# manonkok/Rao-Blackwellized-SLAM-smoothing

Measured on AMD Instinct MI355X. Metric: particle-steps/s (filter) + smoother wall-clock, N=65k T=3k, higher is better.
Workload: dtype f64

## Files before the change

include/rbpf.h:

```cpp
#ifndef RBPF_H_
#define RBPF_H_

#include <stddef.h>
#include <stdint.h>

#ifdef __cplusplus
extern "C" {
#endif

#define RBPF_ABI_VERSION 9

typedef enum {
  RBPF_OK = 0,
  RBPF_ERR_INVALID_ARG = 1,
  RBPF_ERR_UNSUPPORTED = 2,
  RBPF_ERR_HIP = 3,
  RBPF_ERR_NO_DEVICE = 4,
  RBPF_ERR_OUT_OF_MEMORY = 5,
  RBPF_ERR_CHOL_FAILED = 6,
  RBPF_ERR_STATE = 7,
  RBPF_ERR_CALLBACK = 8
} rbpf_status;

typedef enum {
// ... 213 lines not shown
                   int32_t n_p, const double* xn, const double* odo, double dt, const double* Q,
                   const double* z, double* xn_next);
int rbpf_dyn_res_norm(const rbpf_model* model, int32_t n_nonlin, int32_t n_w, int32_t n_odo,
                      int32_t n_p, const double* xnk_t, const double* xn, const double* odo,
                      double dt, const double* Q, double* e_dyn);
int rbpf_sample(int32_t N, const double* w, int32_t n_draws, const double* u, int32_t* ind);
int rbpf_jacobian_phi3d(const rbpf_model* model, int32_t n_p, const double* x,
                        const double* lower, const double* upper, double* J);
int rbpf_chol_weights(int32_t M, int32_t batch, const double* S, const double* e, double jitter,
                      int32_t variant, int32_t reps, double* logw, int32_t* status, double* ms);
int32_t rbpf_chol_refresh_resolve(int32_t model_kind, int32_t n_lin, int32_t n_y, int32_t requested);
int rbpf_chol_sweep_probe(int32_t n, int32_t d, int32_t batch, const double* L, const double* U, const double* V,
                          const double* eta, int32_t reps, double* L_out, double* logw, int32_t* status, double* ms);
int rbpf_quat_helpers(int32_t op, int32_t n, const double* in, double* out);
int rbpf_probe_wave_reduce(const double* in, double* out);

typedef struct {
  int32_t struct_size;
  int32_t m_basis;
  const int32_t* NN;
  double L[3];
  const double* mean;
  const double* V;
  double sigma2;
  const double* var_table;
} rbpf_loc_map;

typedef struct {
  int32_t struct_size;
  int32_t N_P, N_T;
// ... 72 lines not shown
```

rao-blackwellized-slam-smoothing_amd/__init__.py:

```python
from ._build import build, LIBPATH
from ._ffi import (RBPFError, load_library, EXPORTS,
                   RBPF_OK, RBPF_ERR_INVALID_ARG, RBPF_ERR_UNSUPPORTED, RBPF_ERR_HIP, RBPF_ERR_NO_DEVICE,
                   RBPF_ERR_OUT_OF_MEMORY, RBPF_ERR_CHOL_FAILED, RBPF_ERR_STATE, RBPF_ERR_CALLBACK)
from .host import (particleFilter, particleSmoother, particleSmootherInformationForm,
                   DenseMagModel, DenseRadioModel, SparseVisualModel, dense_mag_prior, dense_radio_prior,
                   domain_cartesian_dx, eigenval, PhiloxRNG, ReplayRNG, FilterSession, sample, chol_weights, chol_sweep_probe, quat_helper,
                   GenericDenseModel, particle_filter_external, chol_refresh_in_use,
                   DenseMagMap, particleFilterLocalization, LocalizationSession, loc_workspace_bytes)


def device_count() -> int:
    return int(load_library().rbpf_device_count())
```

rao-blackwellized-slam-smoothing_amd/_ffi.py:

```python
from __future__ import annotations

import ctypes as C
import importlib.util
import os
import sys

from . import _build

c_double_p = C.POINTER(C.c_double)
c_int32_p = C.POINTER(C.c_int32)

RBPF_OK = 0
RBPF_ERR_INVALID_ARG = 1
RBPF_ERR_UNSUPPORTED = 2
RBPF_ERR_HIP = 3
RBPF_ERR_NO_DEVICE = 4
RBPF_ERR_OUT_OF_MEMORY = 5
RBPF_ERR_CHOL_FAILED = 6
RBPF_ERR_STATE = 7
RBPF_ERR_CALLBACK = 8

RBPF_MODEL_DENSE_MAG_6D = 1
RBPF_MODEL_DENSE_RADIO_2DH = 2
RBPF_MODEL_SPARSE_VISUAL_2D = 3
# ... 105 lines not shown

class rbpf_ekf_out(_SizedStructure):
    _fields_ = [("struct_size", C.c_int32), ("reserved", C.c_int32), ("xf_traj", c_double_p), ("qnb_traj", c_double_p),
                ("Pf", c_double_p)]


ABI_STRUCTS = [rbpf_model, rbpf_problem, rbpf_rng, rbpf_options, rbpf_filter_out, rbpf_smoother_out, rbpf_timing, rbpf_callbacks, rbpf_view,
               rbpf_loc_map, rbpf_loc_problem, rbpf_loc_out, rbpf_ekf_problem, rbpf_ekf_out]

EXPORTS = [
    "rbpf_abi_version", "rbpf_abi_sizeof", "rbpf_status_string", "rbpf_last_error", "rbpf_device_count", "rbpf_device_bytes_live",
    "rbpf_particle_filter", "rbpf_particle_smoother",
    "rbpf_filter_create", "rbpf_filter_workspace_bytes", "rbpf_filter_advance", "rbpf_filter_reset", "rbpf_sync",
    "rbpf_filter_finish", "rbpf_filter_tell", "rbpf_filter_schedule", "rbpf_filter_one_launch_flushes", "rbpf_plan_refresh", "rbpf_chol_refresh_resolve", "rbpf_shard_smoother_refresh_reserve", "rbpf_shard_xn_traj", "rbpf_filter_ancestors", "rbpf_filter_step_external", "rbpf_timing_enable", "rbpf_timing_read", "rbpf_destroy",
    "rbpf_philox_fill", "rbpf_meas_model", "rbpf_dyn_model", "rbpf_dyn_res_norm", "rbpf_sample",
    "rbpf_jacobian_phi3d", "rbpf_chol_weights", "rbpf_chol_sweep_probe", "rbpf_quat_helpers", "rbpf_probe_wave_reduce",
    "rbpf_shard_create", "rbpf_shard_views_get", "rbpf_shard_normalise_search", "rbpf_shard_pack", "rbpf_shard_step",
    "rbpf_shard_trajectories", "rbpf_shard_plan", "rbpf_shard_plan_read", "rbpf_shard_normalise_plan",
    "rbpf_stream_get", "rbpf_shard_set_async", "rbpf_shard_finish", "rbpf_shard_set_ancestors",
    "rbpf_shard_smoother_create", "rbpf_shard_smoother_views_get", "rbpf_shard_smoother_begin",
    "rbpf_shard_smoother_normalise", "rbpf_shard_smoother_anc_weights", "rbpf_shard_smoother_anc_sample",
    "rbpf_shard_smoother_refresh_begin", "rbpf_shard_smoother_refresh_pack", "rbpf_shard_smoother_refresh_end",
    "rbpf_shard_smoother_step", "rbpf_shard_smoother_end",
    "rbpf_particle_filter_localization", "rbpf_loc_create", "rbpf_loc_advance", "rbpf_loc_finish", "rbpf_loc_workspace_bytes",
    "rbpf_loc_predict", "rbpf_loc_dyn_model",
    "rbpf_ekf_dense", "rbpf_ekf_workspace_bytes",
]

ABI_VERSION = 9
_lib = None

# ... 66 lines not shown
    lib.rbpf_philox_fill.argtypes = [C.c_uint64, C.c_int32, C.c_int32, C.c_int32, C.c_int32, c_double_p, c_double_p,
                                     c_double_p]
    lib.rbpf_meas_model.argtypes = [C.POINTER(rbpf_model), C.c_int32, C.c_int32, c_double_p, c_double_p]
    lib.rbpf_dyn_model.argtypes = [C.POINTER(rbpf_model), C.c_int32, C.c_int32, C.c_int32, C.c_int32, c_double_p,
                                   c_double_p, C.c_double, c_double_p, c_double_p, c_double_p]
    lib.rbpf_dyn_res_norm.argtypes = [C.POINTER(rbpf_model), C.c_int32, C.c_int32, C.c_int32, C.c_int32, c_double_p,
                                      c_double_p, c_double_p, C.c_double, c_double_p, c_double_p]
    lib.rbpf_sample.argtypes = [C.c_int32, c_double_p, C.c_int32, c_double_p, c_int32_p]
    lib.rbpf_jacobian_phi3d.argtypes = [C.POINTER(rbpf_model), C.c_int32, c_double_p, c_double_p, c_double_p,
                                        c_double_p]
    lib.rbpf_chol_weights.argtypes = [C.c_int32, C.c_int32, c_double_p, c_double_p, C.c_double, C.c_int32, C.c_int32,
                                      c_double_p, c_int32_p, c_double_p]
    lib.rbpf_chol_sweep_probe.argtypes = [C.c_int32, C.c_int32, C.c_int32, c_double_p, c_double_p, c_double_p, c_double_p, C.c_int32,
                                          c_double_p, c_double_p, c_int32_p, c_double_p]
    lib.rbpf_quat_helpers.argtypes = [C.c_int32, C.c_int32, c_double_p, c_double_p]
    lib.rbpf_chol_refresh_resolve.argtypes = [C.c_int32, C.c_int32, C.c_int32, C.c_int32]
    lib.rbpf_chol_refresh_resolve.restype = C.c_int32
    lib.rbpf_particle_filter_localization.argtypes = [C.POINTER(rbpf_loc_map), C.POINTER(rbpf_loc_problem), C.POINTER(rbpf_rng),
                                                      C.POINTER(rbpf_options), C.POINTER(rbpf_loc_out)]
    lib.rbpf_loc_create.argtypes = [C.POINTER(rbpf_loc_map), C.POINTER(rbpf_loc_problem), C.POINTER(rbpf_rng),
                                    C.POINTER(rbpf_options), C.POINTER(C.c_void_p)]
    lib.rbpf_loc_advance.argtypes = [C.c_void_p, C.c_int32]
    lib.rbpf_loc_finish.argtypes = [C.c_void_p, C.POINTER(rbpf_loc_out)]
    lib.rbpf_loc_workspace_bytes.argtypes = [C.POINTER(rbpf_loc_map), C.POINTER(rbpf_loc_problem), C.POINTER(rbpf_options),
                                             C.POINTER(C.c_size_t)]
    lib.rbpf_loc_predict.argtypes = [C.POINTER(rbpf_loc_map), C.c_int32, c_double_p, c_double_p, c_double_p, C.c_int32, c_double_p]
    lib.rbpf_loc_dyn_model.argtypes = [C.c_int32, c_double_p, c_double_p, C.c_double, c_double_p, c_double_p, c_double_p]
    lib.rbpf_ekf_dense.argtypes = [C.POINTER(rbpf_ekf_problem), C.POINTER(rbpf_options), C.POINTER(rbpf_ekf_out)]
    lib.rbpf_ekf_workspace_bytes.argtypes = [C.POINTER(rbpf_ekf_problem), C.POINTER(rbpf_options), C.POINTER(C.c_size_t)]
    _lib = lib
# ... 9 lines not shown
```

rao-blackwellized-slam-smoothing_amd/csrc/rbpf_api.hip:

```cpp
#include "../../include/rbpf.h"
#include "rbpf_internal.hpp"
#include "rbpf_ctx.hpp"
#include "rbpf_sparse.hpp"

#include <cmath>
#include <cstdio>
#include <cstdlib>
#include <cstring>
#include <string>
#include <vector>

namespace rbpf {

thread_local std::string g_last_error;

void set_error(const std::string& s) { g_last_error = s; }

int hip_fail(hipError_t e, const char* what, const char* file, int line) {
  char buf[512];
  snprintf(buf, sizeof(buf), "%s failed: %s (%s:%d)", what, hipGetErrorString(e), file, line);
  g_last_error = buf;
  (void)hipGetLastError();
  return (e == hipErrorOutOfMemory) ? RBPF_ERR_OUT_OF_MEMORY : RBPF_ERR_HIP;
}
// ... 691 lines not shown
  if (c->mdl.kind == RBPF_MODEL_GENERIC_DENSE && (!a.xn_ext || !a.H_ext)) {
    set_error("generic (host-callback) model: advance with rbpf_filter_step_external"); return RBPF_ERR_STATE;
  }
  const bool flushing = lazy && bk.flush && t > 0;
  const bool share = flushing && step_shares_flush(a) && (c->inplace ? c->share_inplace : c->share_flush);
  FlushMode mode = FlushMode::Plain;
  if (flushing && c->inplace) {
    if (!a.order) { set_error("in-place flush without a processing order"); return RBPF_ERR_STATE; }
    int* dst = c->d_ip; int* ph = c->d_ip + N; int* scratch = c->d_ip + 2 * (size_t)N;
    if (share) HIPCHK(launch_share_inplace_plan(N, a.order, A_t, c->base[bk.told], dst, ph, scratch, c->timing_on ? c->d_share_writers : nullptr, c->stream));
    else HIPCHK(launch_inplace_plan(N, a.order, A_t, c->base[bk.told], dst, ph, scratch, c->stream));
    a.dst_slot = dst; a.phase_of = ph;
    mode = share ? FlushMode::InPlaceShared : FlushMode::InPlace;
  } else if (share) {
    int* lead = c->d_share; int* dst = c->d_share + N; int* ph = c->d_share + 2 * (size_t)N;
    HIPCHK(launch_share_plan(N, N, A_t, lead, dst, ph, c->timing_on ? c->d_share_writers : nullptr, c->stream));
    a.dst_slot = dst; a.phase_of = ph;
    mode = FlushMode::Shared;
  }
  a.share_flush = share ? 1 : 0;
  RB_TRY(ctx_arm_distinct(c, a, (size_t)N + 1));
  HIPCHK(launch_propagate(a, c->stream));
  RB_TRY(ctx_launch_step(c, a, bk, mode));

  NormArgs nm;
  nm.N = N; nm.nN = nN; nm.t = t; nm.logw = c->logw + tr; nm.w = c->w + tr; nm.wc = c->wc; nm.xn = X_new;
  nm.traj_max = c->traj_max + (size_t)t * nN; nm.traj_mean = c->traj_mean + (size_t)t * nN;
  nm.iw_max = c->d_flags + 2; nm.lse_out = nullptr;
  nm.parallel_scan = 1;
  if (c->fuse_resample && t + 1 < c->T) {
    int* A_next = c->A + (hist ? (size_t)(t + 1) * N : 0);
    SearchArgs s;
    s.N = N; s.n_draw = N; s.t = t + 1; s.wc = c->wc; s.rng_mode = c->rng_mode; s.k_iter = k_iter;
    s.U = c->d_U ? c->d_U + rng_page + (size_t)t * N : nullptr;
    if (a.u_next) { s.rng_mode = RBPF_RNG_REPLAY; s.U = c->d_unext; }
    s.seed = c->seed; s.ai = A_next; s.overflow = c->d_flags + 1; s.slot0 = 0; s.u_is_scalar = 0;
    s.approx = 1; s.ambiguous = c->d_flags + 4; s.w = c->w + tr; s.wc_exact = c->wc;
    if (N > kSingleWgResampleMaxN)
      HIPCHK(launch_resample_pipeline(nm, &s, c->d_order, c->d_counts, lazy ? c->base[bk.tnew] : nullptr, c->d_rs, c->stream));
    else
      HIPCHK(launch_normalise_resample(nm, s, c->d_order, c->d_counts, c->stream, lazy ? c->base[bk.tnew] : nullptr));
    c->ready_step = t + 1;
  } else if (N > kSingleWgResampleMaxN) {
    HIPCHK(launch_resample_pipeline(nm, nullptr, nullptr, nullptr, nullptr, c->d_rs, c->stream));
  } else {
    HIPCHK(launch_normalise_scan(nm, c->stream));
  }
  return RBPF_OK;
}

int ctx_unpack(rbpf_ctx* c, const int* d_index, int count, double* d_out) {
  const Layout& L = c->lay;
  const int d = c->mdl.d, N = c->N;
  if (c->lazy_depth < 2) {
    HIPCHK(launch_unpack_P(L, d, c->Pt[c->cur], c->Pb[c->cur], c->t > 0 ? c->F[c->cur] : nullptr, d_index, count, d_out, c->stream,
// ... 539 lines not shown
  HIPCHK(hipMemcpy(out, dout, (size_t)n * nout_of[op] * 8, hipMemcpyDeviceToHost));
  return RBPF_OK;
}

int rbpf_probe_wave_reduce(const double* in, double* out) {
  if (!have_device()) { set_error("no HIP device"); return RBPF_ERR_NO_DEVICE; }
  if (!in || !out) { set_error("bad argument"); return RBPF_ERR_INVALID_ARG; }
  DevicePool tmp; double *di = nullptr, *dout = nullptr;
  RB_TRY(tmp.upload(&di, in, 256)); RB_TRY(tmp.alloc(&dout, 4));
  HIPCHK(launch_probe_wave_reduce(di, dout, 0));
  HIPCHK(hipDeviceSynchronize());
  HIPCHK(hipMemcpy(out, dout, 4 * 8, hipMemcpyDeviceToHost));
  return RBPF_OK;
}

int rbpf_jacobian_phi3d(const rbpf_model* model, int32_t n_p, const double* x, const double* lower, const double* upper, double* J) {
  if (!have_device()) { set_error("no HIP device"); return RBPF_ERR_NO_DEVICE; }
  if (!model || model->kind != RBPF_MODEL_DENSE_MAG_6D || !x || !lower || !upper || !J || n_p < 1) { set_error("bad argument"); return RBPF_ERR_INVALID_ARG; }
  ModelDev M; DevicePool tmp; double *dx = nullptr, *dlo = nullptr, *dup = nullptr, *dj = nullptr;
  RB_TRY(model_for_helpers(model, 7, 6, 7, M, tmp));
  RB_TRY(tmp.upload(&dx, x, (size_t)3 * n_p)); RB_TRY(tmp.upload(&dlo, lower, 3)); RB_TRY(tmp.upload(&dup, upper, 3)); RB_TRY(tmp.alloc(&dj, (size_t)9 * M.m * n_p));
  HIPCHK(launch_jacobian_phi3d(M, n_p, dx, dlo, dup, dj, 0));
  HIPCHK(hipDeviceSynchronize());
  HIPCHK(hipMemcpy(J, dj, (size_t)9 * M.m * n_p * 8, hipMemcpyDeviceToHost));
  return RBPF_OK;
}

}
```

rao-blackwellized-slam-smoothing_amd/csrc/rbpf_ctx.hpp:

```cpp
#pragma once
#include "../../include/rbpf.h"
#include "rbpf_internal.hpp"
#include "rbpf_devmem.hpp"

#include <memory>
#include <string>
#include <utility>
#include <vector>

namespace rbpf {

void set_error(const std::string& s);
int hip_fail(hipError_t e, const char* what, const char* file, int line);

#define HIPCHK(expr)                                                          \
  do {                                                                        \
    hipError_t _e = (expr);                                                   \
    if (_e != hipSuccess) return ::rbpf::hip_fail(_e, #expr, __FILE__, __LINE__); \
  } while (0)
#define RB_TRY(x) do { int _s = (x); if (_s != RBPF_OK) return _s; } while (0)

inline bool have_device() {
  int n = 0;
  return hipGetDeviceCount(&n) == hipSuccess && n > 0;
// ... 54 lines not shown
  rbpf_callbacks cb = {nullptr, nullptr, nullptr, nullptr};
  bool has_cb = false;
  std::vector<double> h_xn;
  std::vector<double> h_xn_new, h_dy;
  std::vector<int> h_ai;
  std::vector<double> h_odo, h_Q, h_dt;
  int q_pages = 1, dt_len = 1;
  bool cholQfull_ok = true;
  int drawn_step = -1;
  bool fp32 = false;
  bool inplace = false;
  int* d_ip = nullptr;
  bool share_inplace = false;
  bool share_flush = false;
  int* d_share = nullptr;
  double* d_strip_ws = nullptr; size_t strip_ws_stride = 0;
  unsigned long long* d_share_writers = nullptr;
  long long share_flush_particles = 0;
  long long one_launch_flushes = 0;
  int* d_distinct_mark = nullptr; size_t distinct_keys = 0; unsigned long long* d_distinct_counter = nullptr;
  long long distinct_nominal = 0; int distinct_epoch = 0;
  int hist_slabs = 2;
  double* X = nullptr;
  int* A = nullptr;
  double *logw = nullptr, *w = nullptr, *wc = nullptr;
  double *traj_max = nullptr, *traj_mean = nullptr;
  double* d_scal = nullptr;
  int* d_flags = nullptr;
  int t = 0;
  int overflow_draws = 0;
// ... 88 lines not shown
```

rao-blackwellized-slam-smoothing_amd/csrc/rbpf_internal.hpp:

```cpp
#pragma once
#include <hip/hip_runtime.h>
#include <stdint.h>
#include <stddef.h>
#include <stdlib.h>
#include <atomic>

namespace rbpf {

inline hipError_t lds_opt_in(const void* kernel, int bytes, std::atomic<uint64_t>& done) {
  int dev = 0;
  hipError_t e = hipGetDevice(&dev);
  if (e != hipSuccess) return e;
  const uint64_t bit = 1ull << (dev & 63);
  if (dev < 64 && (done.load(std::memory_order_acquire) & bit)) return hipSuccess;
  e = hipFuncSetAttribute(kernel, hipFuncAttributeMaxDynamicSharedMemorySize, bytes);
  if (e != hipSuccess) return e;
  if (dev < 64) done.fetch_or(bit, std::memory_order_release);
  return hipSuccess;
}

#ifdef RBPF_TUNING
inline const char* tuning_env(const char* key) { return getenv(key); }
#else
inline const char* tuning_env(const char*) { return nullptr; }
// ... 145 lines not shown
bool sym_supported(int n, int d);
size_t sym_strip_doubles(const Layout& lay, int d);
size_t step_sym_lds_bytes(const ModelDev& m, const Layout& lay, int n_sets, int write_base, int extra = 0);
hipError_t launch_step_sym(const StepArgs& a, hipStream_t s);
bool step_sym_shared_one_launch(const StepArgs& a);
hipError_t launch_step_sym_shared(const StepArgs& a, hipStream_t s);
hipError_t launch_probe_wave_reduce(const double* in, double* out, hipStream_t s);

hipError_t launch_propagate(const StepArgs& a, hipStream_t s);
hipError_t launch_step(const StepArgs& a, hipStream_t s);
hipError_t launch_normalise_scan(const NormArgs& a, hipStream_t s);
hipError_t launch_search(const SearchArgs& a, hipStream_t s);
hipError_t launch_cumsum(int N, const double* w, double* wc, hipStream_t s);
hipError_t launch_normalise_resample(const NormArgs& a, const SearchArgs& sa, int* order, int* counts, hipStream_t s,
                                     const int* remap = nullptr);
hipError_t launch_order_large(int n_slots, int range, const int* key, const int* remap, int* order, int* counts, hipStream_t s);
hipError_t launch_order(int n_slots, int range, const int* key, int* order, int* counts, hipStream_t s, const int* remap = nullptr);
hipError_t launch_inplace_plan(int N, const int* order, const int* ai, const int* base, int* dst, int* phase,
                               int* scratch, hipStream_t s);
hipError_t launch_share_inplace_plan(int N, const int* order, const int* ai, const int* base, int* dst, int* phase, int* scratch,
                                     unsigned long long* writers, hipStream_t s);
hipError_t launch_share_plan(int N, int nkeys, const int* ai, int* lead, int* dst, int* phase, unsigned long long* writers, hipStream_t s);
size_t resample_scratch_doubles(int N);
hipError_t launch_resample_pipeline(const NormArgs& nm, const SearchArgs* sa, int* order, int* counts, const int* remap,
                                    double* scratch, hipStream_t s);
hipError_t launch_resample_lse(int N, const double* scratch, double* out, hipStream_t s);
constexpr int kMaxParticles = 1024 * 1024;
constexpr int kSingleWgResampleMaxN = 8192;
hipError_t launch_resample_fixup(const SearchArgs& a, hipStream_t s);

hipError_t launch_pack_P(const Layout& lay, const double* P_colmajor, size_t src_stride, double* Pt,
                         double* Pb, int count, hipStream_t s, int fp32 = 0);
hipError_t launch_unpack_P(const Layout& lay, int d, const double* Pt, const double* Pb, const double* F,
                           const int* index, int count, double* P_colmajor, hipStream_t s, int fp32 = 0);
hipError_t launch_unpack_P_sets(const Layout& lay, int d, const double* Pt, const double* Pb, int n_sets,
                                const double* const* fset, const int* const* fidx, const int* base, const int* index,
                                int count, double* P_colmajor, hipStream_t s, int fp32 = 0);
hipError_t launch_weighted_mean_xl(int N, int n, int ldx, const double* xl, const double* w, double* out,
                                   hipStream_t s);
hipError_t launch_backtrace(int N, int nN, int T, const double* X, const int* A, const int* start_index,
// ... 25 lines not shown
```

rao-blackwellized-slam-smoothing_amd/csrc/rbpf_resample.hip:

```cpp
#include "rbpf_internal.hpp"
#include "rbpf_device.hpp"

namespace rbpf {

constexpr int kRB = 1024;

__device__ inline double blk_sum(double v, double* sred) {
  const int lane = threadIdx.x & 63, wave = threadIdx.x >> 6;
  v = wave_sum(v);
  __syncthreads();
  if (lane == 0) sred[wave] = v;
  __syncthreads();
  double s = sred[0];
  for (int w = 1; w < kRB / 64; ++w) s += sred[w];
  return s;
}

__device__ inline double blk_max(double v, double* sred) {
  const int lane = threadIdx.x & 63, wave = threadIdx.x >> 6;
#pragma unroll
  for (int off = 32; off > 0; off >>= 1) v = fmax(v, __shfl_xor(v, off, 64));
  __syncthreads();
  if (lane == 0) sred[wave] = v;
  __syncthreads();
// ... 18 lines not shown
__global__ __launch_bounds__(kRB) void rs_sumexp_kernel(int N, int B, const double* __restrict__ logw,
                                                        const double* __restrict__ pmax, double* __restrict__ psum) {
  __shared__ double sred[16];
  const double c = global_max(pmax, B, sred);
  const int i = blockIdx.x * kRB + threadIdx.x;
  const double s = blk_sum(i < N ? exp(logw[i] - c) : 0.0, sred);
  if (threadIdx.x == 0) psum[blockIdx.x] = s;
}

__global__ __launch_bounds__(kRB) void rs_weights_kernel(NormArgs a, int B, const double* __restrict__ pmax,
                                                         const double* __restrict__ psum, double* __restrict__ btot,
                                                         double* __restrict__ bparts ) {
  __shared__ double sred[16];
  __shared__ int sidx[16];
  __shared__ double sbc;
  const int tid = threadIdx.x, lane = tid & 63, wave = tid >> 6, N = a.N;
  const double c = global_max(pmax, B, sred);
  if (tid == 0) { double t = 0.0; for (int b = 0; b < B; ++b) t += psum[b]; sbc = c + log(t); }
  __syncthreads();
  const double lse = sbc;
  const int i = blockIdx.x * kRB + tid;
  const double wi = (i < N) ? exp(a.logw[i] - lse) : 0.0;
  if (i < N) a.w[i] = wi;
  double bw = (i < N) ? wi : -1.0;
  int bi = (i < N) ? i : 0x7fffffff;
#pragma unroll
  for (int off = 32; off > 0; off >>= 1) {
    const double ow = __shfl_xor(bw, off, 64);
    const int oi = __shfl_xor(bi, off, 64);
    if (ow > bw || (ow == bw && oi < bi)) { bw = ow; bi = oi; }
  }
  __syncthreads();
  if (lane == 0) { sred[wave] = bw; sidx[wave] = bi; }
// ... 13 lines not shown
  for (int off = 1; off < 64; off <<= 1) {
    const double o = __shfl_up(inc, off, 64);
    if (lane >= off) inc += o;
  }
  __syncthreads();
  if (lane == 63) sred[wave] = inc;
  __syncthreads();
  double woff = 0.0;
  for (int w = 0; w < wave; ++w) woff += sred[w];
  const double lp = woff + inc;
  if (i < N) a.wc[i] = lp;
  if (tid == kRB - 1) btot[blockIdx.x] = lp;
}

__global__ __launch_bounds__(kRB) void rs_offsets_kernel(NormArgs a, int B, const double* __restrict__ btot,
                                                         const double* __restrict__ bparts) {
  __shared__ double sb[1024];
  __shared__ double sp[16][10];
  __shared__ double soff;
  const int tid = threadIdx.x, N = a.N;
  for (int b = tid; b < B; b += kRB) sb[b] = btot[b];
  __syncthreads();
  if (tid == 0) { double t = 0.0; for (int b = 0; b < (int)blockIdx.x; ++b) t += sb[b]; soff = t; }
  __syncthreads();
  const int i = blockIdx.x * kRB + tid;
  if (i < N && blockIdx.x > 0) a.wc[i] = soff + a.wc[i];
  if (blockIdx.x == 0) {
    if (tid < 2 + a.nN) {
      const int q = tid;
      if (q >= 2) {
        double t = 0.0;
        for (int b = 0; b < B; ++b) t += bparts[b * 10 + q];
        sp[0][q] = t;
      }
    }
    if (tid == 0) {
      double gw = bparts[0]; int gi = (int)bparts[1];
      for (int b = 1; b < B; ++b) { const double w = bparts[b * 10]; const int ix = (int)bparts[b * 10 + 1]; if (w > gw || (w == gw && ix < gi)) { gw = w; gi = ix; } }
      if (gi < 0 || gi >= N) gi = 0;
      *a.iw_max = gi;
      sp[1][0] = (double)gi;
    }
    __syncthreads();
    if (tid >= 2 && tid < 2 + a.nN) {
      const int cix = tid - 2, gi = (int)sp[1][0];
      if (a.traj_mean) a.traj_mean[cix] = sp[0][tid];
      if (a.traj_max) a.traj_max[cix] = a.xn[(size_t)cix * N + gi];
    }
  }
}

__global__ void rs_hist_kernel(int N, const int* __restrict__ key, const int* __restrict__ remap, int* __restrict__ counts) {
  const int i = blockIdx.x * blockDim.x + threadIdx.x;
  if (i < N) atomicAdd(&counts[remap ? remap[key[i]] : key[i]], 1);
}

__global__ __launch_bounds__(kRB) void rs_scan_kernel(int N, int* __restrict__ counts) {
  __shared__ int swave[kRB / 64];
  const int tid = threadIdx.x, lane = tid & 63, wave = tid >> 6;
  const int S = (N + kRB - 1) / kRB;
  const int j0 = min(tid * S, N), j1 = min(j0 + S, N);
  constexpr int NBATCH = 8;
  int tot = 0;
  for (int jb = j0; jb < j1; jb += NBATCH) {
    int v[NBATCH];
#pragma unroll
    for (int k = 0; k < NBATCH; ++k) v[k] = counts[min(jb + k, N - 1)];
#pragma unroll
    for (int k = 0; k < NBATCH; ++k) tot += (jb + k < j1) ? v[k] : 0;
// ... 3 lines not shown
  for (int off = 1; off < 64; off <<= 1) { const int o = __shfl_up(inc, off, 64); if (lane >= off) inc += o; }
  if (lane == 63) swave[wave] = inc;
  __syncthreads();
  int run = inc - tot;
  for (int w = 0; w < wave; ++w) run += swave[w];
  for (int jb = j0; jb < j1; jb += NBATCH) {
    int v[NBATCH];
#pragma unroll
    for (int k = 0; k < NBATCH; ++k) v[k] = counts[min(jb + k, N - 1)];
#pragma unroll
    for (int k = 0; k < NBATCH; ++k)
      if (jb + k < j1) { counts[jb + k] = run; run += v[k]; }
  }
}

__global__ void rs_scatter_kernel(int N, const int* __restrict__ key, const int* __restrict__ remap, int* __restrict__ counts,
                                  int* __restrict__ order) {
  const int i = blockIdx.x * blockDim.x + threadIdx.x;
  if (i < N) order[atomicAdd(&counts[remap ? remap[key[i]] : key[i]], 1)] = i;
}

size_t resample_scratch_doubles(int N) { return (size_t)13 * ((N + kRB - 1) / kRB) + 16; }

hipError_t launch_resample_pipeline(const NormArgs& nm, const SearchArgs* sa, int* order, int* counts, const int* remap,
                                    double* scratch, hipStream_t s) {
  const int N = nm.N, B = (N + kRB - 1) / kRB;
  double* pmax = scratch; double* psum = pmax + B; double* btot = psum + B; double* bparts = btot + B;
  hipLaunchKernelGGL(rs_max_kernel, dim3(B), dim3(kRB), 0, s, N, nm.logw, pmax);
  hipLaunchKernelGGL(rs_sumexp_kernel, dim3(B), dim3(kRB), 0, s, N, B, nm.logw, pmax, psum);
  hipLaunchKernelGGL(rs_weights_kernel, dim3(B), dim3(kRB), 0, s, nm, B, pmax, psum, btot, bparts);
  hipLaunchKernelGGL(rs_offsets_kernel, dim3(B), dim3(kRB), 0, s, nm, B, btot, bparts);
  hipError_t e = hipGetLastError();
  if (e != hipSuccess || !sa) return e;
  SearchArgs q = *sa;
  q.scan_depth = B + 32;
  if ((e = launch_search(q, s)) != hipSuccess) return e;
  if (q.approx && (e = launch_resample_fixup(q, s)) != hipSuccess) return e;
  if (order) {
    if ((e = hipMemsetAsync(counts, 0, (size_t)N * sizeof(int), s)) != hipSuccess) return e;
    const int nb = (q.n_draw + 255) / 256;
    hipLaunchKernelGGL(rs_hist_kernel, dim3(nb), dim3(256), 0, s, q.n_draw, q.ai, remap, counts);
    hipLaunchKernelGGL(rs_scan_kernel, dim3(1), dim3(kRB), 0, s, N, counts);
    hipLaunchKernelGGL(rs_scatter_kernel, dim3(nb), dim3(256), 0, s, q.n_draw, q.ai, remap, counts, order);
    e = hipGetLastError();
  }
  return e;
}

__global__ void rs_lse_kernel(int B, const double* __restrict__ pmax, const double* __restrict__ psum, double* __restrict__ out) {
  double c = -INFINITY, t = 0.0;
  for (int b = 0; b < B; ++b) c = fmax(c, pmax[b]);
  for (int b = 0; b < B; ++b) t += psum[b];
  *out = c + log(t);
}

hipError_t launch_resample_lse(int N, const double* scratch, double* out, hipStream_t s) {
  const int B = (N + kRB - 1) / kRB;
  hipLaunchKernelGGL(rs_lse_kernel, dim3(1), dim3(1), 0, s, B, scratch, scratch + B, out);
  return hipGetLastError();
}

hipError_t launch_order_large(int n_slots, int range, const int* key, const int* remap, int* order, int* counts, hipStream_t s) {
  hipError_t e = hipMemsetAsync(counts, 0, (size_t)range * sizeof(int), s);
  if (e != hipSuccess) return e;
  const int nb = (n_slots + 255) / 256;
  hipLaunchKernelGGL(rs_hist_kernel, dim3(nb), dim3(256), 0, s, n_slots, key, remap, counts);
  hipLaunchKernelGGL(rs_scan_kernel, dim3(1), dim3(kRB), 0, s, range, counts);
  hipLaunchKernelGGL(rs_scatter_kernel, dim3(nb), dim3(256), 0, s, n_slots, key, remap, counts, order);
  return hipGetLastError();
}

__global__ void ip_mark_kernel(int N, const int* __restrict__ ai, const int* __restrict__ base, int* __restrict__ has,
                               int* __restrict__ nzp) {
  const int i = blockIdx.x * blockDim.x + threadIdx.x;
  if (i < N) { const int s = base[ai[i]]; has[s] = 1; nzp[s] = 1; }
}

__global__ void ip_free_kernel(int N, const int* __restrict__ has, const int* __restrict__ nzp, int* __restrict__ freelist) {
  const int f = blockIdx.x * blockDim.x + threadIdx.x;
  if (f < N && !has[f]) freelist[f - nzp[f]] = f;
}

__global__ void ip_assign_kernel(int N, const int* __restrict__ order, const int* __restrict__ ai, const int* __restrict__ base,
                                 const int* __restrict__ nzp, const int* __restrict__ freelist, int* __restrict__ dst,
                                 int* __restrict__ phase) {
  const int b = blockIdx.x * blockDim.x + threadIdx.x;
  if (b >= N) return;
  const int i = order[b];
  const int s = base[ai[i]];
  const int prev = (b > 0) ? base[ai[order[b - 1]]] : -1;
  const bool first = (s != prev);
  dst[i] = first ? s : freelist[b - nzp[s] - 1];
  phase[i] = first ? 1 : 0;
}

__global__ void share_fill_kernel(int N, int* lead) {
  const int i = blockIdx.x * blockDim.x + threadIdx.x;
  if (i < N) lead[i] = 0x7fffffff;
}
__global__ void share_min_kernel(int N, const int* __restrict__ ai, int* lead) {
  const int i = blockIdx.x * blockDim.x + threadIdx.x;
  if (i < N) atomicMin(&lead[ai[i]], i);
}
__global__ void share_assign_kernel(int N, const int* __restrict__ ai, const int* __restrict__ lead, int* __restrict__ dst,
                                    int* __restrict__ phase, unsigned long long* writers) {
  const int i = blockIdx.x * blockDim.x + threadIdx.x;
  const bool w = i < N && lead[ai[i]] == i;
  if (i < N) { dst[i] = lead[ai[i]]; phase[i] = w ? 1 : 0; }
  const unsigned long long m = __ballot(w);
  if (writers && (threadIdx.x & 63) == 0 && m) atomicAdd(writers, (unsigned long long)__popcll(m));
}

hipError_t launch_share_plan(int N, int nkeys, const int* ai, int* lead, int* dst, int* phase, unsigned long long* writers, hipStream_t s) {
  const int nb = (N + 255) / 256;
  hipLaunchKernelGGL(share_fill_kernel, dim3((nkeys + 255) / 256), dim3(256), 0, s, nkeys, lead);
  hipLaunchKernelGGL(share_min_kernel, dim3(nb), dim3(256), 0, s, N, ai, lead);
  hipLaunchKernelGGL(share_assign_kernel, dim3(nb), dim3(256), 0, s, N, ai, lead, dst, phase, writers);
  return hipGetLastError();
}

__global__ void sip_fill_kernel(int N, int* lead, int* leadbase, int* has, int* nzp) {
  const int i = blockIdx.x * blockDim.x + threadIdx.x;
  if (i < N) { lead[i] = 0x7fffffff; leadbase[i] = 0x7fffffff; has[i] = 0; nzp[i] = 0; }
}
__global__ void sip_mark_kernel(int N, const int* __restrict__ ai, const int* __restrict__ base, int* lead, int* __restrict__ has, int* __restrict__ nzp) {
  const int i = blockIdx.x * blockDim.x + threadIdx.x;
  if (i < N) { atomicMin(&lead[ai[i]], i); const int s = base[ai[i]]; has[s] = 1; nzp[s] = 1; }
}
__global__ void sip_first_kernel(int N, const int* __restrict__ order, const int* __restrict__ ai, const int* __restrict__ base,
                                 const int* __restrict__ lead, int* leadbase) {
// ... 67 lines not shown
```

rao-blackwellized-slam-smoothing_amd/host.py:

```python
from __future__ import annotations

import ctypes as C
import math
from dataclasses import dataclass
from typing import Callable, Optional

import numpy as np

from . import _ffi
from ._ffi import RBPFError, check, load_library


def domain_cartesian_dx(m: int, d: int, LL):
    LL = np.atleast_2d(np.asarray(LL, dtype=np.float64))
    L = (LL.max(axis=0) - LL.min(axis=0)) / 2.0 if LL.shape[0] > 1 else LL.ravel().copy()
    if L.size != d:
        raise ValueError("LL must have d columns")
    counts = np.ceil(m ** (1.0 / d) * L / L.min()).astype(np.int64)
    axes = [np.arange(1, c + 1, dtype=np.int64) for c in counts]
    grid = np.stack([g.ravel() for g in np.meshgrid(*axes, indexing="ij")], axis=1)
    lam = eigenval(grid, L)
    order = np.argsort(lam, kind="stable")[:m]
    return L, grid[order].astype(np.int32)

# ... 690 lines not shown
    lib = load_library()
    L = np.asfortranarray(np.asarray(L, dtype=np.float64))
    U = np.asfortranarray(np.asarray(U, dtype=np.float64))
    V = np.asfortranarray(np.asarray(V, dtype=np.float64))
    eta = np.ascontiguousarray(np.asarray(eta, dtype=np.float64))
    d, n = U.shape
    assert L.shape == (n + 1, n + 1) and V.shape == (d, n) and eta.shape == (d,)
    Lo = np.zeros((n + 1, n + 1), order="F")
    logw = np.zeros(1)
    status = np.zeros(1, dtype=np.int32)
    ms = np.zeros(1)
    check(lib.rbpf_chol_sweep_probe(n, d, int(batch), _dp(L), _dp(U), _dp(V), _dp(eta), int(reps), _dp(Lo), _dp(logw), _ip(status), _dp(ms)))
    return Lo, float(logw[0]), int(status[0]), float(ms[0])


class FilterSession:

    def __init__(self, model, odometry, y, x0_nonLin, x0_lin, P0_lin, Q, R, N_P, dt, rng=None, keep_history=False,
                 trace=False, lazy_depth=0, inplace=0, storage="fp64"):
        self.lib = load_library()
        self.model = model
        self.prob = _Problem(model, odometry, y, x0_nonLin, x0_lin, P0_lin, Q, R, N_P, dt)
        self.blk, self._rng = _rng_block(rng, self.prob.N_P, self.prob.N_T, model.nw, 1)
        self.opt = _ffi.rbpf_options(keep_history=1 if keep_history else 0, trace=1 if trace else 0, fix_p_mean=0,
                                     lazy_depth=int(lazy_depth), jitter=0.0, inplace=int(inplace),
                                     storage=_storage_code(storage))
        self.mdesc = model.descriptor()
        self.ctx = C.c_void_p()
        check(self.lib.rbpf_filter_create(C.byref(self.mdesc), C.byref(self.prob.c), C.byref(self.blk),
                                          C.byref(self.opt), C.byref(self.ctx)))
# ... 335 lines not shown
```

Baseline: 5.976 million.

## Parallelise counting-sort scan and fold resample zero-fills into offsets kernel

Replaces the single-workgroup scan in the large-N resample counting sort with a multi-block scan. Per-block totals are rescanned in LDS inside the scatter kernel. The hipMemset of counts and the share-plan lead fill move into the existing offsets kernel, so one memset and one fill launch are dropped per step. The offsets kernel also stages bparts through LDS for its block-0 reduction, psum is staged in LDS, and a probe entry point for the ordering routine is added. The cost is extra state tracking whether lead was prefilled, which must stay consistent across flush modes.

```diff
diff --git a/include/rbpf.h b/include/rbpf.h
--- a/include/rbpf.h
+++ b/include/rbpf.h
@@ -251,6 +251,7 @@
                           const double* eta, int32_t reps, double* L_out, double* logw, int32_t* status, double* ms);
 int rbpf_quat_helpers(int32_t op, int32_t n, const double* in, double* out);
 int rbpf_probe_wave_reduce(const double* in, double* out);
+int rbpf_order_probe(int32_t n_slots, int32_t range, const int32_t* key, const int32_t* remap, int32_t* order_out);
 
 typedef struct {
   int32_t struct_size;
diff --git a/rao-blackwellized-slam-smoothing_amd/__init__.py b/rao-blackwellized-slam-smoothing_amd/__init__.py
--- a/rao-blackwellized-slam-smoothing_amd/__init__.py
+++ b/rao-blackwellized-slam-smoothing_amd/__init__.py
@@ -4,7 +4,7 @@
                    RBPF_ERR_OUT_OF_MEMORY, RBPF_ERR_CHOL_FAILED, RBPF_ERR_STATE, RBPF_ERR_CALLBACK)
 from .host import (particleFilter, particleSmoother, particleSmootherInformationForm,
                    DenseMagModel, DenseRadioModel, SparseVisualModel, dense_mag_prior, dense_radio_prior,
-                   domain_cartesian_dx, eigenval, PhiloxRNG, ReplayRNG, FilterSession, sample, chol_weights, chol_sweep_probe, quat_helper,
+                   domain_cartesian_dx, eigenval, PhiloxRNG, ReplayRNG, FilterSession, sample, chol_weights, chol_sweep_probe, order_probe, quat_helper,
                    GenericDenseModel, particle_filter_external, chol_refresh_in_use,
                    DenseMagMap, particleFilterLocalization, LocalizationSession, loc_workspace_bytes)
 
diff --git a/rao-blackwellized-slam-smoothing_amd/_ffi.py b/rao-blackwellized-slam-smoothing_amd/_ffi.py
--- a/rao-blackwellized-slam-smoothing_amd/_ffi.py
+++ b/rao-blackwellized-slam-smoothing_amd/_ffi.py
@@ -143,7 +143,7 @@
     "rbpf_filter_create", "rbpf_filter_workspace_bytes", "rbpf_filter_advance", "rbpf_filter_reset", "rbpf_sync",
     "rbpf_filter_finish", "rbpf_filter_tell", "rbpf_filter_schedule", "rbpf_filter_one_launch_flushes", "rbpf_plan_refresh", "rbpf_chol_refresh_resolve", "rbpf_shard_smoother_refresh_reserve", "rbpf_shard_xn_traj", "rbpf_filter_ancestors", "rbpf_filter_step_external", "rbpf_timing_enable", "rbpf_timing_read", "rbpf_destroy",
     "rbpf_philox_fill", "rbpf_meas_model", "rbpf_dyn_model", "rbpf_dyn_res_norm", "rbpf_sample",
-    "rbpf_jacobian_phi3d", "rbpf_chol_weights", "rbpf_chol_sweep_probe", "rbpf_quat_helpers", "rbpf_probe_wave_reduce",
+    "rbpf_jacobian_phi3d", "rbpf_chol_weights", "rbpf_chol_sweep_probe", "rbpf_quat_helpers", "rbpf_probe_wave_reduce", "rbpf_order_probe",
     "rbpf_shard_create", "rbpf_shard_views_get", "rbpf_shard_normalise_search", "rbpf_shard_pack", "rbpf_shard_step",
     "rbpf_shard_trajectories", "rbpf_shard_plan", "rbpf_shard_plan_read", "rbpf_shard_normalise_plan",
     "rbpf_stream_get", "rbpf_shard_set_async", "rbpf_shard_finish", "rbpf_shard_set_ancestors",
@@ -240,6 +240,8 @@
     lib.rbpf_chol_sweep_probe.argtypes = [C.c_int32, C.c_int32, C.c_int32, c_double_p, c_double_p, c_double_p, c_double_p, C.c_int32,
                                           c_double_p, c_double_p, c_int32_p, c_double_p]
     lib.rbpf_quat_helpers.argtypes = [C.c_int32, C.c_int32, c_double_p, c_double_p]
+    if hasattr(lib, "rbpf_order_probe"):
+        lib.rbpf_order_probe.argtypes = [C.c_int32, C.c_int32, c_int32_p, c_int32_p, c_int32_p]
     lib.rbpf_chol_refresh_resolve.argtypes = [C.c_int32, C.c_int32, C.c_int32, C.c_int32]
     lib.rbpf_chol_refresh_resolve.restype = C.c_int32
     lib.rbpf_particle_filter_localization.argtypes = [C.POINTER(rbpf_loc_map), C.POINTER(rbpf_loc_problem), C.POINTER(rbpf_rng),
diff --git a/rao-blackwellized-slam-smoothing_amd/csrc/rbpf_api.hip b/rao-blackwellized-slam-smoothing_amd/csrc/rbpf_api.hip
--- a/rao-blackwellized-slam-smoothing_amd/csrc/rbpf_api.hip
+++ b/rao-blackwellized-slam-smoothing_amd/csrc/rbpf_api.hip
@@ -729,7 +729,8 @@
     mode = share ? FlushMode::InPlaceShared : FlushMode::InPlace;
   } else if (share) {
     int* lead = c->d_share; int* dst = c->d_share + N; int* ph = c->d_share + 2 * (size_t)N;
-    HIPCHK(launch_share_plan(N, N, A_t, lead, dst, ph, c->timing_on ? c->d_share_writers : nullptr, c->stream));
+    HIPCHK(launch_share_plan(N, N, A_t, lead, dst, ph, c->timing_on ? c->d_share_writers : nullptr, c->stream, c->share_lead_filled));
+    c->share_lead_filled = false;
     a.dst_slot = dst; a.phase_of = ph;
     mode = FlushMode::Shared;
   }
@@ -751,9 +752,10 @@
     if (a.u_next) { s.rng_mode = RBPF_RNG_REPLAY; s.U = c->d_unext; }
     s.seed = c->seed; s.ai = A_next; s.overflow = c->d_flags + 1; s.slot0 = 0; s.u_is_scalar = 0;
     s.approx = 1; s.ambiguous = c->d_flags + 4; s.w = c->w + tr; s.wc_exact = c->wc;
-    if (N > kSingleWgResampleMaxN)
-      HIPCHK(launch_resample_pipeline(nm, &s, c->d_order, c->d_counts, lazy ? c->base[bk.tnew] : nullptr, c->d_rs, c->stream));
-    else
+    if (N > kSingleWgResampleMaxN) {
+      HIPCHK(launch_resample_pipeline(nm, &s, c->d_order, c->d_counts, lazy ? c->base[bk.tnew] : nullptr, c->d_rs, c->stream, c->d_share));
+      c->share_lead_filled = c->d_share != nullptr;
+    } else
       HIPCHK(launch_normalise_resample(nm, s, c->d_order, c->d_counts, c->stream, lazy ? c->base[bk.tnew] : nullptr));
     c->ready_step = t + 1;
   } else if (N > kSingleWgResampleMaxN) {
@@ -1323,6 +1325,23 @@
   return RBPF_OK;
 }
 
+int rbpf_order_probe(int32_t n_slots, int32_t range, const int32_t* key, const int32_t* remap, int32_t* order_out) {
+  if (!have_device()) { set_error("no HIP device"); return RBPF_ERR_NO_DEVICE; }
+  if (n_slots < 1 || range < 1 || !key || !order_out) { set_error("bad argument"); return RBPF_ERR_INVALID_ARG; }
+  if (range > kMaxParticles) { set_error("rbpf_order_probe: range above 2^20"); return RBPF_ERR_INVALID_ARG; }
+  for (int i = 0; i < n_slots; ++i) {
+    const int k = key[i];
+    if (k < 0 || k >= range || (remap && (remap[k] < 0 || remap[k] >= range))) { set_error("rbpf_order_probe: key outside the range"); return RBPF_ERR_INVALID_ARG; }
+  }
+  DevicePool tmp; int *dk = nullptr, *dr = nullptr, *dord = nullptr, *dcnt = nullptr;
+  RB_TRY(tmp.upload(&dk, key, (size_t)n_slots)); RB_TRY(tmp.alloc(&dord, (size_t)n_slots)); RB_TRY(tmp.alloc(&dcnt, order_large_scratch_ints(range)));
+  if (remap) RB_TRY(tmp.upload(&dr, remap, (size_t)range));
+  HIPCHK(launch_order_large(n_slots, range, dk, dr, dord, dcnt, 0));
+  HIPCHK(hipDeviceSynchronize());
+  HIPCHK(hipMemcpy(order_out, dord, (size_t)n_slots * 4, hipMemcpyDeviceToHost));
+  return RBPF_OK;
+}
+
 int rbpf_jacobian_phi3d(const rbpf_model* model, int32_t n_p, const double* x, const double* lower, const double* upper, double* J) {
   if (!have_device()) { set_error("no HIP device"); return RBPF_ERR_NO_DEVICE; }
   if (!model || model->kind != RBPF_MODEL_DENSE_MAG_6D || !x || !lower || !upper || !J || n_p < 1) { set_error("bad argument"); return RBPF_ERR_INVALID_ARG; }
diff --git a/rao-blackwellized-slam-smoothing_amd/csrc/rbpf_ctx.hpp b/rao-blackwellized-slam-smoothing_amd/csrc/rbpf_ctx.hpp
--- a/rao-blackwellized-slam-smoothing_amd/csrc/rbpf_ctx.hpp
+++ b/rao-blackwellized-slam-smoothing_amd/csrc/rbpf_ctx.hpp
@@ -92,6 +92,7 @@
   bool share_inplace = false;
   bool share_flush = false;
   int* d_share = nullptr;
+  bool share_lead_filled = false;
   double* d_strip_ws = nullptr; size_t strip_ws_stride = 0;
   unsigned long long* d_share_writers = nullptr;
   long long share_flush_particles = 0;
diff --git a/rao-blackwellized-slam-smoothing_amd/csrc/rbpf_internal.hpp b/rao-blackwellized-slam-smoothing_amd/csrc/rbpf_internal.hpp
--- a/rao-blackwellized-slam-smoothing_amd/csrc/rbpf_internal.hpp
+++ b/rao-blackwellized-slam-smoothing_amd/csrc/rbpf_internal.hpp
@@ -183,16 +183,18 @@
 hipError_t launch_cumsum(int N, const double* w, double* wc, hipStream_t s);
 hipError_t launch_normalise_resample(const NormArgs& a, const SearchArgs& sa, int* order, int* counts, hipStream_t s,
                                      const int* remap = nullptr);
+size_t order_large_scratch_ints(int range);
 hipError_t launch_order_large(int n_slots, int range, const int* key, const int* remap, int* order, int* counts, hipStream_t s);
 hipError_t launch_order(int n_slots, int range, const int* key, int* order, int* counts, hipStream_t s, const int* remap = nullptr);
 hipError_t launch_inplace_plan(int N, const int* order, const int* ai, const int* base, int* dst, int* phase,
                                int* scratch, hipStream_t s);
 hipError_t launch_share_inplace_plan(int N, const int* order, const int* ai, const int* base, int* dst, int* phase, int* scratch,
                                      unsigned long long* writers, hipStream_t s);
-hipError_t launch_share_plan(int N, int nkeys, const int* ai, int* lead, int* dst, int* phase, unsigned long long* writers, hipStream_t s);
+hipError_t launch_share_plan(int N, int nkeys, const int* ai, int* lead, int* dst, int* phase, unsigned long long* writers, hipStream_t s,
+                             bool lead_filled = false);
 size_t resample_scratch_doubles(int N);
 hipError_t launch_resample_pipeline(const NormArgs& nm, const SearchArgs* sa, int* order, int* counts, const int* remap,
-                                    double* scratch, hipStream_t s);
+                                    double* scratch, hipStream_t s, int* lead_fill = nullptr);
 hipError_t launch_resample_lse(int N, const double* scratch, double* out, hipStream_t s);
 constexpr int kMaxParticles = 1024 * 1024;
 constexpr int kSingleWgResampleMaxN = 8192;
diff --git a/rao-blackwellized-slam-smoothing_amd/csrc/rbpf_resample.hip b/rao-blackwellized-slam-smoothing_amd/csrc/rbpf_resample.hip
--- a/rao-blackwellized-slam-smoothing_amd/csrc/rbpf_resample.hip
+++ b/rao-blackwellized-slam-smoothing_amd/csrc/rbpf_resample.hip
@@ -4,6 +4,7 @@
 namespace rbpf {
 
 constexpr int kRB = 1024;
+constexpr int kShareNoChild = 0x7fffffff;
 
 __device__ inline double blk_sum(double v, double* sred) {
   const int lane = threadIdx.x & 63, wave = threadIdx.x >> 6;
@@ -56,9 +57,11 @@
   __shared__ double sred[16];
   __shared__ int sidx[16];
   __shared__ double sbc;
+  __shared__ double sps[kRB];
   const int tid = threadIdx.x, lane = tid & 63, wave = tid >> 6, N = a.N;
+  for (int b = tid; b < B; b += kRB) sps[b] = psum[b];
   const double c = global_max(pmax, B, sred);
-  if (tid == 0) { double t = 0.0; for (int b = 0; b < B; ++b) t += psum[b]; sbc = c + log(t); }
+  if (tid == 0) { double t = 0.0; for (int b = 0; b < B; ++b) t += sps[b]; sbc = c + log(t); }
   __syncthreads();
   const double lse = sbc;
   const int i = blockIdx.x * kRB + tid;
@@ -102,7 +105,8 @@
 }
 
 __global__ __launch_bounds__(kRB) void rs_offsets_kernel(NormArgs a, int B, const double* __restrict__ btot,
-                                                         const double* __restrict__ bparts) {
+                                                         const double* __restrict__ bparts, int* __restrict__ zero,
+                                                         int* __restrict__ lead_fill) {
   __shared__ double sb[1024];
   __shared__ double sp[16][10];
   __shared__ double soff;
@@ -113,27 +117,35 @@
   __syncthreads();
   const int i = blockIdx.x * kRB + tid;
   if (i < N && blockIdx.x > 0) a.wc[i] = soff + a.wc[i];
+  if (i < N && zero) zero[i] = 0;
+  if (i < N && lead_fill) lead_fill[i] = kShareNoChild;
   if (blockIdx.x == 0) {
-    if (tid < 2 + a.nN) {
-      const int q = tid;
-      if (q >= 2) {
-        double t = 0.0;
-        for (int b = 0; b < B; ++b) t += bparts[b * 10 + q];
-        sp[0][q] = t;
-      }
+    constexpr int kStage = 1024 / 10;
+    double t = 0.0, gw = 0.0; int gi = 0;
+    for (int b0 = 0; b0 < B; b0 += kStage) {
+      const int nb = min(kStage, B - b0);
+      __syncthreads();
+      for (int j = tid; j < nb * 10; j += kRB) sb[j] = bparts[b0 * 10 + j];
+      __syncthreads();
+      if (tid >= 2 && tid < 2 + a.nN)
+        for (int b = 0; b < nb; ++b) t += sb[b * 10 + tid];
+      if (tid == 0)
+        for (int b = 0; b < nb; ++b) {
+          const double w = sb[b * 10]; const int ix = (int)sb[b * 10 + 1];
+          if (b0 + b == 0 || w > gw || (w == gw && ix < gi)) { gw = w; gi = ix; }
+        }
     }
+    if (tid >= 2 && tid < 2 + a.nN) sp[0][tid] = t;
     if (tid == 0) {
-      double gw = bparts[0]; int gi = (int)bparts[1];
-      for (int b = 1; b < B; ++b) { const double w = bparts[b * 10]; const int ix = (int)bparts[b * 10 + 1]; if (w > gw || (w == gw && ix < gi)) { gw = w; gi = ix; } }
       if (gi < 0 || gi >= N) gi = 0;
       *a.iw_max = gi;
       sp[1][0] = (double)gi;
     }
     __syncthreads();
     if (tid >= 2 && tid < 2 + a.nN) {
-      const int cix = tid - 2, gi = (int)sp[1][0];
+      const int cix = tid - 2, gmax = (int)sp[1][0];
       if (a.traj_mean) a.traj_mean[cix] = sp[0][tid];
-      if (a.traj_max) a.traj_max[cix] = a.xn[(size_t)cix * N + gi];
+      if (a.traj_max) a.traj_max[cix] = a.xn[(size_t)cix * N + gmax];
     }
   }
 }
@@ -141,6 +153,22 @@
 __global__ void rs_hist_kernel(int N, const int* __restrict__ key, const int* __restrict__ remap, int* __restrict__ counts) {
   const int i = blockIdx.x * blockDim.x + threadIdx.x;
   if (i < N) atomicAdd(&counts[remap ? remap[key[i]] : key[i]], 1);
+}
+
+__global__ __launch_bounds__(kRB) void rs_scan_blocks_kernel(int range, int* __restrict__ counts, int* __restrict__ btot) {
+  __shared__ int swave[kRB / 64];
+  const int tid = threadIdx.x, lane = tid & 63, wave = tid >> 6;
+  const int j = blockIdx.x * kRB + tid;
+  const int v = (j < range) ? counts[j] : 0;
+  int inc = v;
+#pragma unroll
+  for (int off = 1; off < 64; off <<= 1) { const int o = __shfl_up(inc, off, 64); if (lane >= off) inc += o; }
+  if (lane == 63) swave[wave] = inc;
+  __syncthreads();
+  int woff = 0;
+  for (int w = 0; w < wave; ++w) woff += swave[w];
+  if (j < range) counts[j] = woff + inc - v;
+  if (tid == kRB - 1) btot[blockIdx.x] = woff + inc;
 }
 
 __global__ __launch_bounds__(kRB) void rs_scan_kernel(int N, int* __restrict__ counts) {
@@ -174,36 +202,66 @@
   }
 }
 
-__global__ void rs_scatter_kernel(int N, const int* __restrict__ key, const int* __restrict__ remap, int* __restrict__ counts,
-                                  int* __restrict__ order) {
-  const int i = blockIdx.x * blockDim.x + threadIdx.x;
-  if (i < N) order[atomicAdd(&counts[remap ? remap[key[i]] : key[i]], 1)] = i;
+constexpr int kScatterThreads = 256;
+constexpr int kOrderMaxBlocks = 4 * kScatterThreads;
+__global__ __launch_bounds__(kScatterThreads) void rs_scatter_kernel(int N, int nbt, const int* __restrict__ key,
+                                                                     const int* __restrict__ remap, int* __restrict__ counts,
+                                                                     const int* __restrict__ btot, int* __restrict__ order) {
+  __shared__ int sboff[kOrderMaxBlocks];
+  __shared__ int swave[kScatterThreads / 64];
+  const int tid = threadIdx.x, lane = tid & 63, wave = tid >> 6;
+  int v[4], tot = 0;
+#pragma unroll
+  for (int k = 0; k < 4; ++k) { v[k] = (4 * tid + k < nbt) ? btot[4 * tid + k] : 0; tot += v[k]; }
+  int inc = tot;
+#pragma unroll
+  for (int off = 1; off < 64; off <<= 1) { const int o = __shfl_up(inc, off, 64); if (lane >= off) inc += o; }
+  if (lane == 63) swave[wave] = inc;
+  __syncthreads();
+  int run = inc - tot;
+  for (int w = 0; w < wave; ++w) run += swave[w];
+#pragma unroll
+  for (int k = 0; k < 4; ++k) { sboff[4 * tid + k] = run; run += v[k]; }
+  __syncthreads();
+  const int i = blockIdx.x * kScatterThreads + tid;
+  if (i < N) {
+    const int k = remap ? remap[key[i]] : key[i];
+    order[sboff[k >> 10] + atomicAdd(&counts[k], 1)] = i;
+  }
+}
+
+static_assert(kRB == 1024, "rs_scatter_kernel takes the block of a key as key >> 10");
+static_assert(kMaxParticles <= kOrderMaxBlocks * kRB, "the block totals of the counting sort must fit one LDS scan");
+
+size_t order_large_scratch_ints(int range) { return (size_t)range + (size_t)((range + kRB - 1) / kRB); }
+
+static hipError_t launch_scan_scatter(int n_slots, int range, const int* key, const int* remap, int* order, int* counts, hipStream_t s) {
+  const int nbt = (range + kRB - 1) / kRB, nb = (n_slots + kScatterThreads - 1) / kScatterThreads;
+  if (range < 1 || nbt > kOrderMaxBlocks) return hipErrorInvalidValue;
+  int* btot = counts + range;
+  hipLaunchKernelGGL(rs_hist_kernel, dim3(nb), dim3(kScatterThreads), 0, s, n_slots, key, remap, counts);
+  hipLaunchKernelGGL(rs_scan_blocks_kernel, dim3(nbt), dim3(kRB), 0, s, range, counts, btot);
+  hipLaunchKernelGGL(rs_scatter_kernel, dim3(nb), dim3(kScatterThreads), 0, s, n_slots, nbt, key, remap, counts, btot, order);
+  return hipGetLastError();
 }
 
 size_t resample_scratch_doubles(int N) { return (size_t)13 * ((N + kRB - 1) / kRB) + 16; }
 
 hipError_t launch_resample_pipeline(const NormArgs& nm, const SearchArgs* sa, int* order, int* counts, const int* remap,
-                                    double* scratch, hipStream_t s) {
+                                    double* scratch, hipStream_t s, int* lead_fill) {
   const int N = nm.N, B = (N + kRB - 1) / kRB;
   double* pmax = scratch; double* psum = pmax + B; double* btot = psum + B; double* bparts = btot + B;
   hipLaunchKernelGGL(rs_max_kernel, dim3(B), dim3(kRB), 0, s, N, nm.logw, pmax);
   hipLaunchKernelGGL(rs_sumexp_kernel, dim3(B), dim3(kRB), 0, s, N, B, nm.logw, pmax, psum);
   hipLaunchKernelGGL(rs_weights_kernel, dim3(B), dim3(kRB), 0, s, nm, B, pmax, psum, btot, bparts);
-  hipLaunchKernelGGL(rs_offsets_kernel, dim3(B), dim3(kRB), 0, s, nm, B, btot, bparts);
+  hipLaunchKernelGGL(rs_offsets_kernel, dim3(B), dim3(kRB), 0, s, nm, B, btot, bparts, (sa && order) ? counts : nullptr, lead_fill);
   hipError_t e = hipGetLastError();
   if (e != hipSuccess || !sa) return e;
   SearchArgs q = *sa;
   q.scan_depth = B + 32;
   if ((e = launch_search(q, s)) != hipSuccess) return e;
   if (q.approx && (e = launch_resample_fixup(q, s)) != hipSuccess) return e;
-  if (order) {
-    if ((e = hipMemsetAsync(counts, 0, (size_t)N * sizeof(int), s)) != hipSuccess) return e;
-    const int nb = (q.n_draw + 255) / 256;
-    hipLaunchKernelGGL(rs_hist_kernel, dim3(nb), dim3(256), 0, s, q.n_draw, q.ai, remap, counts);
-    hipLaunchKernelGGL(rs_scan_kernel, dim3(1), dim3(kRB), 0, s, N, counts);
-    hipLaunchKernelGGL(rs_scatter_kernel, dim3(nb), dim3(256), 0, s, q.n_draw, q.ai, remap, counts, order);
-    e = hipGetLastError();
-  }
+  if (order) e = launch_scan_scatter(q.n_draw, N, q.ai, remap, order, counts, s);
   return e;
 }
 
@@ -221,13 +279,10 @@
 }
 
 hipError_t launch_order_large(int n_slots, int range, const int* key, const int* remap, int* order, int* counts, hipStream_t s) {
+  if (range < 1 || (range + kRB - 1) / kRB > kOrderMaxBlocks) return hipErrorInvalidValue;
   hipError_t e = hipMemsetAsync(counts, 0, (size_t)range * sizeof(int), s);
   if (e != hipSuccess) return e;
-  const int nb = (n_slots + 255) / 256;
-  hipLaunchKernelGGL(rs_hist_kernel, dim3(nb), dim3(256), 0, s, n_slots, key, remap, counts);
-  hipLaunchKernelGGL(rs_scan_kernel, dim3(1), dim3(kRB), 0, s, range, counts);
-  hipLaunchKernelGGL(rs_scatter_kernel, dim3(nb), dim3(256), 0, s, n_slots, key, remap, counts, order);
-  return hipGetLastError();
+  return launch_scan_scatter(n_slots, range, key, remap, order, counts, s);
 }
 
 __global__ void ip_mark_kernel(int N, const int* __restrict__ ai, const int* __restrict__ base, int* __restrict__ has,
@@ -256,7 +311,7 @@
 
 __global__ void share_fill_kernel(int N, int* lead) {
   const int i = blockIdx.x * blockDim.x + threadIdx.x;
-  if (i < N) lead[i] = 0x7fffffff;
+  if (i < N) lead[i] = kShareNoChild;
 }
 __global__ void share_min_kernel(int N, const int* __restrict__ ai, int* lead) {
   const int i = blockIdx.x * blockDim.x + threadIdx.x;
@@ -271,9 +326,10 @@
   if (writers && (threadIdx.x & 63) == 0 && m) atomicAdd(writers, (unsigned long long)__popcll(m));
 }
 
-hipError_t launch_share_plan(int N, int nkeys, const int* ai, int* lead, int* dst, int* phase, unsigned long long* writers, hipStream_t s) {
+hipError_t launch_share_plan(int N, int nkeys, const int* ai, int* lead, int* dst, int* phase, unsigned long long* writers, hipStream_t s,
+                             bool lead_filled) {
   const int nb = (N + 255) / 256;
-  hipLaunchKernelGGL(share_fill_kernel, dim3((nkeys + 255) / 256), dim3(256), 0, s, nkeys, lead);
+  if (!lead_filled) hipLaunchKernelGGL(share_fill_kernel, dim3((nkeys + 255) / 256), dim3(256), 0, s, nkeys, lead);
   hipLaunchKernelGGL(share_min_kernel, dim3(nb), dim3(256), 0, s, N, ai, lead);
   hipLaunchKernelGGL(share_assign_kernel, dim3(nb), dim3(256), 0, s, N, ai, lead, dst, phase, writers);
   return hipGetLastError();
diff --git a/rao-blackwellized-slam-smoothing_amd/host.py b/rao-blackwellized-slam-smoothing_amd/host.py
--- a/rao-blackwellized-slam-smoothing_amd/host.py
+++ b/rao-blackwellized-slam-smoothing_amd/host.py
@@ -728,6 +728,17 @@
     return Lo, float(logw[0]), int(status[0]), float(ms[0])
 
 
+def order_probe(key, range_, remap=None):
+    lib = load_library()
+    key = np.ascontiguousarray(np.asarray(key, dtype=np.int32))
+    if remap is not None:
+        remap = np.ascontiguousarray(np.asarray(remap, dtype=np.int32))
+        assert remap.shape == (int(range_),)
+    order = np.full(key.shape[0], -1, dtype=np.int32)
+    check(lib.rbpf_order_probe(key.shape[0], int(range_), _ip(key), _ip(remap) if remap is not None else None, _ip(order)))
+    return order
+
+
 class FilterSession:
 
     def __init__(self, model, odometry, y, x0_nonLin, x0_lin, P0_lin, Q, R, N_P, dt, rng=None, keep_history=False,
```

Result: no change. 5.975 million (-0.0%).
